# megvii-research/OccDepth

Measured on AMD Instinct MI355X. Metric: frames/sec forward, SemanticKITTI stereo->256x256x32 voxels, higher is better.
Workload: dtype f32 storage and accumulate; matrix arithmetic as 3x bf16 split (hi + mid + lo of both operands, six v_mfma_f32_32x32x16_bf16 per K step; error vs float64 tested within 1.5x of the exact-fp32 kernels', measured 0.8-1.1x) in the head convolutions (K2s3), the small-volume 3x3x3 convolutions and transpo

## Files before the change

include/occdepth_amd.h:

```cpp
#ifndef OCCDEPTH_AMD_H
#define OCCDEPTH_AMD_H

#include <stdint.h>

#ifdef __cplusplus
extern "C" {
#endif

#define OCCD_OK 0
#define OCCD_EINVAL (-1)
#define OCCD_ELAUNCH (-2)
#define OCCD_ENOMEM (-3)

#define OCCD_MAX_VIEWS 4
#define OCCD_MAX_SCALES 4

#define OCCD_ACT_NONE 0
#define OCCD_ACT_RELU 1
#define OCCD_ACT_SIGMOID 2
#define OCCD_ACT_RELU_PRE 3

int occd_abi_version(void);
const char* occd_strerror(int code);

// ... 230 lines not shown
                                    int32_t ths, int32_t act, float slope, int32_t res_first, void* stream);

typedef struct occd_wino_args {
    const float* x;
    const float* upk;
    const float* shift;
    const float* res;
    float* y;
    int32_t batch, cin, cout, H, W;
    int32_t act, res_first, tile_hint;
    float slope;
} occd_wino_args;
int64_t occd_wino_packed_floats(int32_t cout, int32_t cin);
int occd_wino_pack_weights(const float* w, const float* scale, float* upk, int32_t cout, int32_t cin, void* stream);
int occd_wino_conv3x3_fwd(const occd_wino_args* a, void* stream);

int occd_dwconv2d_bwd_data_nchw(const float* gy, const float* w, float* dx, int32_t batch, int32_t C, int32_t H,
                                int32_t W, int32_t k, int32_t stride, int32_t pad_top, int32_t pad_left, int32_t Ho,
                                int32_t Wo, void* stream);
int64_t occd_dwconv2d_bwd_weight_workspace_floats(int32_t batch, int32_t C, int32_t k, int32_t Ho, int32_t Wo);
int occd_dwconv2d_bwd_weight_nchw(const float* x, const float* gy, float* dw, float* workspace, int32_t batch, int32_t C,
                                  int32_t H, int32_t W, int32_t k, int32_t stride, int32_t pad_top, int32_t pad_left,
                                  int32_t Ho, int32_t Wo, void* stream);
int32_t occd_dwconv2d_pool_blocks(int32_t Ho, int32_t Wo);
int occd_dwconv2d_pool_nchw(const float* x, const float* w, const float* scale, const float* shift, float* y,
                            float* pool_part, int32_t batch, int32_t C, int32_t H, int32_t W, int32_t k,
                            int32_t stride, int32_t pad_top, int32_t pad_left, int32_t Ho, int32_t Wo,
                            int32_t act, int64_t x_plane_stride, void* stream);
int occd_plane_reduce(const float* a, const float* b, float* out, int64_t planes, int64_t S, void* stream);
int occd_se_bwd(const float* gg, const float* gate, const float* sums, const float* r, const float* w_reduce,
// ... 249 lines not shown
```

occdepth_amd/csrc/prof.cpp:

```cpp
#include <map>
#include <set>
#include <utility>
#include <mutex>
#include <string>
#include <vector>
#include <cstring>
#include "common.h"

namespace {
struct Rec {
    hipEvent_t e0, e1;
    std::string tag;
    double flops, bytes;
};
std::mutex g_mu;
bool g_on = false;
std::string g_tag;
std::string g_tag_kind;
std::vector<Rec> g_recs;
std::vector<hipEvent_t> g_pool;

hipEvent_t get_event() {
    if (!g_pool.empty()) {
        hipEvent_t e = g_pool.back();
// ... 77 lines not shown
        it->second.ms += ms;
        it->second.flops += r.flops;
        it->second.bytes += r.bytes;
        g_pool.push_back(r.e0);
        g_pool.push_back(r.e1);
    }
    g_recs.clear();
    int n = 0;
    for (auto& kv : agg) {
        if (rows && n < max_rows) rows[n] = kv.second;
        ++n;
    }
    return n;
}

extern "C" int occd_abi_version(void) { return 20; }

extern "C" const char* occd_strerror(int code) {
    switch (code) {
        case OCCD_OK: return "ok";
        case OCCD_EINVAL: return "invalid argument or unsupported geometry";
        case OCCD_ELAUNCH: return "HIP launch/runtime error";
        case OCCD_ENOMEM: return "tile does not fit in LDS";
        default: return "unknown error";
    }
}
```

occdepth_amd/csrc/wino_conv2d.hip:

```cpp
#include <type_traits>
#include "device.h"

namespace {

struct WinoP {
    const float* x;
    const float* upk;
    const float* shift;
    const float* res;
    float* y;
    int B, Cin, Cout, H, W;
    int chunks, nblk, wg_ty, wg_tx, nwg;
    int act, res_first;
    float slope;
};

template <int TWV, int EXP = 0>
__global__ void __launch_bounds__(512, 2) wino3x3_kernel(const WinoP p) {
    constexpr int RW = 32 / TWV;
    constexpr int WGR = 4 * RW;
    constexpr int PR = 2 * WGR + 2;
    constexpr int PC = 2 * TWV + 2;
    constexpr int RS = TWV == 16 ? 48 : 68;
    constexpr int PLANE = PR * RS;
    constexpr int NEL = 8 * PLANE;
    constexpr int NDMA = (NEL + 511) / 512;
    constexpr int PBUF = NDMA * 512;
    constexpr int UBUF = 16 * 256;
    extern __shared__ __attribute__((aligned(16))) float lds[];

// ... 129 lines not shown
            if (EXP != 1 && c + 2 < p.chunks) issue_chunk(c + 2);
            block(pn, (c + 1) & 1, 0, ub, vb, ua, va);
        }
        const int lb = (p.chunks - 1) & 1;
        const float* pl = lds + lb * PBUF + pbase;
        block(pl, lb, 1, ua, va, ub, vb);
        block(pl, lb, 2, ub, vb, ua, va);
        block(pl, lb, 3, ua, va, ub, vb);
        mfma4(ub, vb, 0);
        mfma4(ub, vb, 4);
    };
    if (h0) k_loop(std::integral_constant<int, 0>{});
    else k_loop(std::integral_constant<int, 1>{});
    __syncthreads();

    float* const xchg = lds;
    auto xwrite = [&](auto hc) {
        constexpr int H = decltype(hc)::value;
        constexpr bool h0 = H == 0;
        float* mine = xchg + ((pr * 2 + H) * 64) * 64 + lane;
#pragma unroll
        for (int k = 0; k < 8; ++k)
#pragma unroll
            for (int r8 = 0; r8 < 8; ++r8) mine[(k * 8 + r8) * 64] = h0 ? acc[k][8 + r8] : acc[k][r8];
    };
    if (h0) xwrite(std::integral_constant<int, 0>{});
    else xwrite(std::integral_constant<int, 1>{});
    __syncthreads();
    auto finish = [&](auto hc) {
    constexpr int H = decltype(hc)::value;
    constexpr bool h0 = H == 0;
    const float* theirs = xchg + ((pr * 2 + (1 - H)) * 64) * 64 + lane;

    const int oy0 = 2 * (ty0 + lr), ox = 2 * (tx0 + lc);
    const bool pair = ox + 1 < p.W && (p.W & 1) == 0;
#pragma unroll
    for (int r8 = 0; r8 < 8; ++r8) {
        __builtin_amdgcn_sched_barrier(0);
        const int r = H * 8 + r8;
        const int co = nb * 32 + 8 * (r >> 2) + 4 * kk + (r & 3);
        float m[4][4];
#pragma unroll
        for (int k = 0; k < 8; ++k) {
            const float own = h0 ? acc[k][r8] : acc[k][8 + r8];
            const float oth = theirs[(k * 8 + r8) * 64];
            m[k >> 2][k & 3] = h0 ? own : oth;
            m[2 + (k >> 2)][k & 3] = h0 ? oth : own;
        }
        float s[2][4];
#pragma unroll
        for (int j = 0; j < 4; ++j) {
            s[0][j] = m[0][j] + m[1][j] + m[2][j];
            s[1][j] = m[1][j] - m[2][j] - m[3][j];
        }
        if (co >= p.Cout || ox >= p.W) continue;
        const float sh = p.shift != nullptr ? p.shift[co] : 0.f;
#pragma unroll
        for (int a = 0; a < 2; ++a) {
            const int oy = oy0 + a;
            if (oy >= p.H) continue;
            float y0 = s[a][0] + s[a][1] + s[a][2] + sh;
            float y1 = s[a][1] - s[a][2] - s[a][3] + sh;
            const size_t o = (((size_t)b * p.Cout + co) * p.H + oy) * p.W + ox;
            float r0 = 0.f, r1 = 0.f;
            if (p.res != nullptr) {
                r0 = p.res[o];
                if (ox + 1 < p.W) r1 = p.res[o + 1];
            }
            if (p.res_first) { y0 += r0; y1 += r1; }
            y0 = act2d_exact(y0, p.act, p.slope);
            y1 = act2d_exact(y1, p.act, p.slope);
            if (!p.res_first) { y0 += r0; y1 += r1; }
            if (pair) {
                *(f32x2*)(p.y + o) = f32x2{y0, y1};
            } else {
                p.y[o] = y0;
                if (ox + 1 < p.W) p.y[o + 1] = y1;
            }
        }
    }
    };
    if (h0) finish(std::integral_constant<int, 0>{});
    else finish(std::integral_constant<int, 1>{});
}

__global__ void wino_pack_kernel(const float* __restrict__ w, const float* __restrict__ scale, float* __restrict__ upk,
                                 int cout, int cin, int nblk, long total) {
    const long i = (long)blockIdx.x * blockDim.x + threadIdx.x;
    if (i >= total) return;
    const int j = i & 3, lane = (i >> 2) & 63;
    long t = i >> 8;
    const int blk = t % nblk; t /= nblk;
    const int rec = t & 15;
    const int chunk = (int)(t >> 4);
    const int q = rec >> 2, hh = (rec >> 1) & 1, part = rec & 1;
    const int xi = 8 * hh + 4 * part + j;
    const int co = blk * 32 + (lane & 31), ci = chunk * 8 + (lane >> 5) * 4 + q;
    float out = 0.f;
    if (co < cout && ci < cin) {
        const double G[4][3] = {{1, 0, 0}, {0.5, 0.5, 0.5}, {0.5, -0.5, 0.5}, {0, 0, 1}};
        const float* g = w + ((size_t)co * cin + ci) * 9;
        const int a = xi >> 2, bcol = xi & 3;
        double s = 0.0;
#pragma unroll
        for (int m = 0; m < 3; ++m)
#pragma unroll
            for (int n = 0; n < 3; ++n) s += G[a][m] * (double)g[m * 3 + n] * G[bcol][n];
        if (scale != nullptr) s *= (double)scale[co];
        out = (float)s;
    }
    upk[i] = out;
}

template <int TWV, int EXP = 0>
int launch_wino(const WinoP& p, hipStream_t st) {
    constexpr int RW = 32 / TWV, PR = 2 * 4 * RW + 2, RS = TWV == 16 ? 48 : 68;
    constexpr int PBUF = (8 * PR * RS + 511) / 512 * 512;
    size_t lds = ((size_t)2 * PBUF + 2 * 16 * 256) * sizeof(float);
    const size_t xchg = (size_t)4 * 2 * 64 * 64 * sizeof(float);
    if (lds < xchg) lds = xchg;
    if (occd::ensure_big_lds(reinterpret_cast<const void*>(wino3x3_kernel<TWV, EXP>)) != OCCD_OK) return OCCD_ELAUNCH;
    hipLaunchKernelGGL((wino3x3_kernel<TWV, EXP>), dim3((unsigned)p.nwg), dim3(512), lds, st, p);
    return occd::check_launch();
}

}

extern "C" {

int64_t occd_wino_packed_floats(int32_t cout, int32_t cin) {
    if (cout < 1 || cin < 1) return OCCD_EINVAL;
    return (int64_t)((cin + 7) / 8) * 16 * ((cout + 31) / 32) * 256;
}

int occd_wino_pack_weights(const float* w, const float* scale, float* upk, int32_t cout, int32_t cin, void* stream) {
    if (w == nullptr || upk == nullptr || cout < 1 || cin < 1) return OCCD_EINVAL;
    const long total = occd_wino_packed_floats(cout, cin);
    hipLaunchKernelGGL(wino_pack_kernel, dim3((unsigned)((total + 255) / 256)), dim3(256), 0, (hipStream_t)stream, w,
                       scale, upk, cout, cin, (cout + 31) / 32, total);
    return occd::check_launch();
}

int occd_wino_conv3x3_fwd(const occd_wino_args* a, void* stream) {
    if (a == nullptr || a->x == nullptr || a->upk == nullptr || a->y == nullptr) return OCCD_EINVAL;
    if (a->batch < 1 || a->cin < 1 || a->cout < 1 || a->H < 1 || a->W < 1) return OCCD_EINVAL;
    if (a->act < 0 || a->act > 3) return OCCD_EINVAL;
    if ((double)a->cin * a->H * a->W >= 2147483648.0) return OCCD_EINVAL;
    WinoP p{};
    p.x = a->x; p.upk = a->upk; p.shift = a->shift; p.res = a->res; p.y = a->y;
    p.B = a->batch; p.Cin = a->cin; p.Cout = a->cout; p.H = a->H; p.W = a->W;
    p.chunks = (a->cin + 7) / 8;
    p.nblk = (a->cout + 31) / 32;
    p.act = a->act; p.res_first = a->res_first; p.slope = a->slope;
    const int th = (a->H + 1) / 2, tw = (a->W + 1) / 2;
    const int exp_mode = a->tile_hint / 100;
    const int hint = a->tile_hint % 100;
    int twv = hint == 16 || hint == 32 ? hint : 0;
    if (twv == 0) {
        const long w16 = (long)((tw + 15) / 16) * 16 * ((th + 7) / 8) * 8;
        const long w32 = (long)((tw + 31) / 32) * 32 * ((th + 3) / 4) * 4;
        twv = w32 <= w16 ? 32 : 16;
    }
    const int wgr = twv == 16 ? 8 : 4;
    p.wg_tx = (tw + twv - 1) / twv;
    p.wg_ty = (th + wgr - 1) / wgr;
    const long nwg = (long)p.nblk * p.wg_tx * p.wg_ty * p.B;
    if (nwg > 0x7fffffffL) return OCCD_EINVAL;
    p.nwg = (int)nwg;
    const double tiles = (double)p.B * th * tw;
    occd::ProfScope prof("wino_conv3x3", (hipStream_t)stream, 2.0 * 16 * tiles * p.chunks * 8 * p.nblk * 32,
                         4.0 * p.B * ((double)p.Cin + p.Cout) * p.H * p.W);
#ifdef OCCD_WINO_DEV_VARIANTS
    if (exp_mode == 1) return twv == 16 ? launch_wino<16, 1>(p, (hipStream_t)stream) : launch_wino<32, 1>(p, (hipStream_t)stream);
    if (exp_mode == 2) return twv == 16 ? launch_wino<16, 2>(p, (hipStream_t)stream) : launch_wino<32, 2>(p, (hipStream_t)stream);
#else
    (void)exp_mode;
#endif
    return twv == 16 ? launch_wino<16>(p, (hipStream_t)stream) : launch_wino<32>(p, (hipStream_t)stream);
}

}
```

occdepth_amd/fused.py:

```python
import os

import torch

from . import hip
from .hip import ACT_NONE, ACT_RELU, ACT_RELU_PRE, ACT_SIGMOID, Vox


_warned_eval_with_grad = False


def needs_autograd(module):
    if module.training:
        return True
    if torch.is_grad_enabled():
        global _warned_eval_with_grad
        if not _warned_eval_with_grad:
            _warned_eval_with_grad = True
            import warnings
            warnings.warn("occdepth_amd: eval-mode forward with autograd enabled runs the differentiable ATen path; "
                          "wrap inference in torch.no_grad() to take the HIP eval path", stacklevel=3)
        return True
    return False


# ... 23 lines not shown
    b = bn.bias.float() if bn.bias is not None else torch.zeros_like(inv)
    scale = g * inv
    return scale, b - bn.running_mean.float() * scale


def bn_affine_cached(bn):
    key = _stamp(bn)
    cached = getattr(bn, "_occd_affine", None)
    if cached is None or cached[0] != key:
        scale, shift = _bn_affine(bn, bn.num_features, bn.running_mean.device)
        cached = (key, scale.contiguous(), shift.contiguous())
        bn._occd_affine = cached
    return cached[1], cached[2]


def wino_fused_operands(owner, conv, bn):
    key = _stamp(conv, bn)
    cache = owner.__dict__.setdefault("_fused_cache", {})
    hit = cache.get(id(conv))
    if hit is None or hit[0] != key:
        scale, shift = bn_affine_cached(bn)
        if conv.bias is not None:
            shift = shift + scale * conv.bias.detach().float()
        hit = (key, hip.wino_pack_weights(conv.weight, scale), shift.contiguous())
        cache[id(conv)] = hit
    return hit[1:]


def _pad_bias(bias, cout):
    out = torch.zeros(hip.round_up(cout, 32), device=bias.device, dtype=torch.float32)
    out[:cout] = bias
    return out


def _parse_bf16x3(v):
    v = (v or "0").strip().lower()
    if v in ("0", "", "off", "false"):
        return False
    if v in ("1", "all", "on", "true"):
# ... 336 lines not shown
```

occdepth_amd/hip.py:

```python
import ctypes
import os
from ctypes import POINTER, Structure, c_char, c_char_p, c_double, c_float, c_int32, c_int64, c_uint8, c_void_p

import torch

_HERE = os.path.dirname(os.path.abspath(__file__))
LIB_PATH = os.path.join(_HERE, "libocc_hip.so")

MAX_VIEWS = 4
MAX_SCALES = 4
ACT_NONE, ACT_RELU, ACT_SIGMOID, ACT_RELU_PRE = 0, 1, 2, 3
ABI_VERSION = 20

_c_float_p = POINTER(c_float)


class Conv3dArgs(Structure):
    _fields_ = [
        ("inp", c_void_p), ("wpk", c_void_p), ("bias", c_void_p), ("res1", c_void_p), ("res2", c_void_p),
        ("out", c_void_p),
        ("batch", c_int32),
        ("X", c_int32), ("Y", c_int32), ("Z", c_int32),
        ("cin", c_int32), ("in_cs", c_int32), ("in_coff", c_int32),
        ("cout", c_int32), ("out_cs", c_int32), ("out_coff", c_int32),
        ("res1_cs", c_int32), ("res1_coff", c_int32), ("res2_cs", c_int32), ("res2_coff", c_int32),
        ("kx", c_int32), ("ky", c_int32), ("kz", c_int32),
        ("sx", c_int32), ("sy", c_int32), ("sz", c_int32),
# ... 164 lines not shown
                                        c_int32, c_void_p]),
    "occd_affine_act_nchw": (c_int32, [c_void_p, c_void_p, c_void_p, c_void_p, c_void_p, c_int32, c_int32, c_int64,
                                       c_int32, c_float, c_int32, c_void_p]),
    "occd_dwconv2d_nchw": (c_int32, [c_void_p, c_void_p, c_void_p, c_void_p, c_void_p] + [c_int32] * 11 + [c_void_p]),
    "occd_upsample_bilinear_cat_nchw": (c_int32, [c_void_p, c_void_p, c_void_p] + [c_int32] * 7 + [c_void_p]),
    "occd_swish_bwd": (c_int32, [c_void_p, c_void_p, c_void_p, c_int64, c_void_p]),
    "occd_upconv_gather_skip_nchw": (c_int32, [c_void_p] * 5 + [c_int32] * 7 + [c_int64, c_int64, ctypes.c_float, c_void_p]),
    "occd_upconv_gather_nchw": (c_int32, [c_void_p, c_void_p] + [c_int32] * 6 + [c_int64, c_int64, c_void_p]),
    "occd_wino_input_transform_nchw": (c_int32, [c_void_p, c_void_p, c_int32, c_int32, c_int32, c_int32, c_int32, c_int32,
                                                 c_void_p]),
    "occd_wino_output_transform_nchw": (c_int32, [c_void_p, c_void_p, c_void_p, c_void_p, c_void_p, c_int32, c_int32,
                                                  c_int32, c_int32, c_int32, c_int32, c_int32, c_float, c_int32, c_void_p]),
    "occd_wino_packed_floats": (c_int64, [c_int32, c_int32]),
    "occd_wino_pack_weights": (c_int32, [c_void_p, c_void_p, c_void_p, c_int32, c_int32, c_void_p]),
    "occd_wino_conv3x3_fwd": (c_int32, [POINTER(WinoArgs), c_void_p]),
    "occd_softmax_nchw": (c_int32, [c_void_p, c_void_p, c_int32, c_int32, c_int64, c_void_p]),
    "occd_dwconv2d_bwd_data_nchw": (c_int32, [c_void_p, c_void_p, c_void_p] + [c_int32] * 10 + [c_void_p]),
    "occd_dwconv2d_bwd_weight_workspace_floats": (c_int64, [c_int32] * 5),
    "occd_dwconv2d_bwd_weight_nchw": (c_int32, [c_void_p] * 4 + [c_int32] * 10 + [c_void_p]),
    "occd_dwconv2d_pool_blocks": (c_int32, [c_int32, c_int32]),
    "occd_dwconv2d_pool_nchw": (c_int32, [c_void_p] * 6 + [c_int32] * 11 + [c_int64, c_void_p]),
    "occd_se_gate": (c_int32, [c_void_p] * 7 + [c_int32, c_int32, c_int32, c_int32, c_int64, c_void_p]),
    "occd_pw_packed_floats": (c_int64, [c_int32, c_int32]),
    "occd_pw_pack_weights": (c_int32, [c_void_p, c_void_p, c_void_p, c_int32, c_int32, c_void_p]),
    "occd_pw_conv_fwd": (c_int32, [POINTER(PwArgs), c_void_p]),
    "occd_project_voxels": (c_int32, [c_void_p, c_void_p, c_void_p, c_double] + [c_int32] * 5
                            + [c_void_p, c_void_p, c_void_p, c_void_p]),
    "occd_argmax_channels": (c_int32, [c_void_p, c_int64, c_int32, c_int32, c_int32, c_void_p, c_void_p, c_void_p]),
    "occd_cascade_tail_fwd": (c_int32, [c_void_p, c_void_p, c_void_p] + [c_int32] * 8 + [c_void_p]),
    "occd_conv3d_wgrad_workspace_floats": (c_int64, [POINTER(WgradArgs)]),
# ... 1078 lines not shown
def wino_pack_weights(w, scale=None):
    cout, cin = w.shape[0], w.shape[1]
    if tuple(w.shape[2:]) != (3, 3):
        raise RuntimeError("wino_pack_weights needs a (Cout, Cin, 3, 3) weight")
    n = load().occd_wino_packed_floats(cout, cin)
    if n <= 0:
        raise RuntimeError("occd_wino_packed_floats: bad shape")
    wc = w.detach().float().contiguous()
    upk = torch.empty(n, device=w.device, dtype=torch.float32)
    sc = scale.detach().float().contiguous() if scale is not None else None
    _check(load().occd_wino_pack_weights(_f32(wc, "w"), _f32(sc, "scale") if sc is not None else None,
                                         _f32(upk, "upk"), cout, cin, _stream()), "occd_wino_pack_weights")
    return upk


def conv2d_3x3_fused(x, upk, cout, shift=None, act=None, slope=0.01, res=None, res_first=False, tile_hint=0, out=None):
    if not x.is_contiguous():
        x = x.contiguous()
    B, cin, H, W = x.shape
    y = torch.empty((B, cout, H, W), device=x.device, dtype=torch.float32) if out is None else out
    if res is not None and not res.is_contiguous():
        res = res.contiguous()
    a = WinoArgs()
    a.x, a.upk, a.y = _f32(x, "x"), _f32(upk, "upk"), _f32(y, "y")
    a.shift = _f32(shift, "shift") if shift is not None else None
    a.res = _f32(res, "res") if res is not None else None
    a.batch, a.cin, a.cout, a.H, a.W = B, cin, cout, H, W
    a.act, a.res_first, a.tile_hint, a.slope = ACT2D[act], 1 if res_first else 0, int(tile_hint), float(slope)
    if upk.numel() != load().occd_wino_packed_floats(cout, cin):
        raise RuntimeError("packed Winograd weights do not match (cout, cin)")
    if _PROFILING:
        set_tag("%d>%d @%dx%dx%d" % (cin, cout, B, H, W))
    _check(load().occd_wino_conv3x3_fwd(ctypes.byref(a), _stream()), "occd_wino_conv3x3_fwd")
    return y


def pw_pack_weights(w, scale=None):
    cout, cin = w.shape[0], w.shape[1]
    n = load().occd_pw_packed_floats(cout, cin)
    if n <= 0 or w.numel() != cout * cin:
        raise RuntimeError("pw_pack_weights needs a (Cout, Cin[, 1, 1]) weight")
    wc = w.detach().float().reshape(cout, cin).contiguous()
    wpk = torch.empty(n, device=w.device, dtype=torch.float32)
    sc = scale.detach().float().contiguous() if scale is not None else None
    _check(load().occd_pw_pack_weights(_f32(wc, "w"), _f32(sc, "scale") if sc is not None else None, _f32(wpk, "wpk"),
                                       cout, cin, _stream()), "occd_pw_pack_weights")
    return wpk

# ... 744 lines not shown
```

occdepth_amd/models/unet2d.py:

```python
import os

import torch
import torch.nn as nn
import torch.nn.functional as F

from .. import autograd3d as _ag
from .. import hip
from .. import fused as _fused
from ..fused import _stamp, bn_affine_cached, needs_autograd, wino_fused_operands
from .efficientnet import EfficientNet, pw_operands, pw_wins

MODEL_NAME = "tf_efficientnet_b3_ns"
MODEL_CHANNELS = {
    "tf_efficientnet_b3_ns": [3, 24, 32, 48, 136],
    "tf_efficientnet_b4_ns": [3, 24, 32, 56, 160],
    "tf_efficientnet_b5_ns": [3, 32, 40, 64, 176],
    "tf_efficientnet_b7_ns": [3, 32, 48, 80, 224],
}
NUM_FEATURES = {
    "tf_efficientnet_b3_ns": 1536,
    "tf_efficientnet_b4_ns": 1792,
    "tf_efficientnet_b5_ns": 2048,
    "tf_efficientnet_b7_ns": 2560,
}
# ... 46 lines not shown
            U, scale, shift = self._wino_operands(conv, bn)
            return hip.conv2d_3x3_winograd(f, U, scale, shift, "leaky", act.negative_slope)
        if self.WINOGRAD and C >= self.WINOGRAD_HIRES_MIN_CIN and B * H * W <= self.WINOGRAD_HIRES_PIXELS:
            U, scale, shift = self._wino_operands(conv, bn)
            per_row = 16.0 * B * ((W + 1) // 2) * (C + conv.out_channels) * 4
            rows = max(1, int(self.WINOGRAD_STRIP_MB * 2 ** 20 / per_row))
            return hip.conv2d_3x3_winograd(f, U, scale, shift, "leaky", act.negative_slope, strip_rows=rows)
        return hip.affine_act(conv(f), *bn_affine_cached(bn), "leaky", slope=act.negative_slope)

    UPCONV = os.environ.get("OCCDEPTH_UPCONV", "1") == "1"
    UPCONV_LIB_BELOW = int(os.environ.get("OCCDEPTH_UPCONV_LIB_BELOW", str(1 << 62)))
    UPCONV_FOLD_BELOW = int(os.environ.get("OCCDEPTH_UPCONV_FOLD_BELOW", "0"))
    UPCONV_FUSE_SKIP = os.environ.get("OCCDEPTH_UPCONV_FUSE_SKIP", "1") == "1"

    def _upconv_operands(self, conv, bn, cup):
        key = (_stamp(conv, bn), cup)
        hit = self.__dict__.get("_upconv_cache")
        if hit is None or hit[0] != key:
            scale, shift = bn_affine_cached(bn)
            if conv.bias is not None:
                shift = shift + scale * conv.bias.detach().float()
            w = conv.weight.detach().float()
            cout = w.shape[0]
            w9 = (w[:, :cup] * scale.view(-1, 1, 1, 1)).permute(2, 3, 0, 1).reshape(9 * cout, cup).contiguous()
            wskip = (w[:, cup:] * scale.view(-1, 1, 1, 1)).contiguous()
            hit = (key, hip.pw_pack_weights(w9), hip.matmul_operand(w9, "a"),
                   hip.wino_pack_weights(w[:, cup:].contiguous(), scale), shift.contiguous(), wskip)
            self.__dict__["_upconv_cache"] = hit
        return hit[1:]

    @staticmethod
    def _tap_planes(shape, device):
        return hip.padded_rows(shape, device) if hip.GEMM_X3 else None

    def _first_conv_upconv(self, x, skip, conv, bn, act):
        wpk9, w9, upk_skip, shift, wskip = self._upconv_operands(conv, bn, x.shape[1])
        cout = conv.out_channels
        B, cup, h, w = x.shape
        if B > 1 and B * h * w <= self.UPCONV_FOLD_BELOW:
            z = hip.matmul(w9, x.permute(1, 0, 2, 3).reshape(cup, B * h * w),
                           out=self._tap_planes((9 * cout, B * h * w), x.device)).view(9 * cout, B, h, w)
            batch_inner = True
# ... 210 lines not shown
```

Before: 60.68.

## Add fp16 two-term split Winograd 3x3 conv kernel with per-channel scaling

Adds a Winograd F(2,3) 3x3 convolution kernel that splits the transformed input and weights into fp16 hi/lo pairs. It runs three f16 MFMAs per step instead of the existing fp32-emulating path, with per-output-channel power-of-two scaling to keep the fp16 ranges safe. The old epilogue is factored into a shared exchange/store helper that can apply that scale factor. The fp16 path is on by default through OCCDEPTH_WINO_SPLIT, and a heuristic falls back to the fp32 kernel when the grid is too small to fill the CUs. Packing weights now does a blocking host sync to reject non-finite values, and the fp16 split may lose some accuracy relative to the fp32 path.

```diff
diff --git a/include/occdepth_amd.h b/include/occdepth_amd.h
--- a/include/occdepth_amd.h
+++ b/include/occdepth_amd.h
@@ -268,6 +268,10 @@
 int64_t occd_wino_packed_floats(int32_t cout, int32_t cin);
 int occd_wino_pack_weights(const float* w, const float* scale, float* upk, int32_t cout, int32_t cin, void* stream);
 int occd_wino_conv3x3_fwd(const occd_wino_args* a, void* stream);
+
+int64_t occd_wino_packed_f16x2_bytes(int32_t cout, int32_t cin);
+int occd_wino_pack_weights_f16x2(const float* w, const float* scale, void* upk, int32_t cout, int32_t cin, void* stream);
+int occd_wino_conv3x3_f16x2_fwd(const occd_wino_args* a, void* stream);
 
 int occd_dwconv2d_bwd_data_nchw(const float* gy, const float* w, float* dx, int32_t batch, int32_t C, int32_t H,
                                 int32_t W, int32_t k, int32_t stride, int32_t pad_top, int32_t pad_left, int32_t Ho,
diff --git a/occdepth_amd/csrc/prof.cpp b/occdepth_amd/csrc/prof.cpp
--- a/occdepth_amd/csrc/prof.cpp
+++ b/occdepth_amd/csrc/prof.cpp
@@ -115,7 +115,7 @@
     return n;
 }
 
-extern "C" int occd_abi_version(void) { return 20; }
+extern "C" int occd_abi_version(void) { return 21; }
 
 extern "C" const char* occd_strerror(int code) {
     switch (code) {
diff --git a/occdepth_amd/csrc/wino_conv2d.hip b/occdepth_amd/csrc/wino_conv2d.hip
--- a/occdepth_amd/csrc/wino_conv2d.hip
+++ b/occdepth_amd/csrc/wino_conv2d.hip
@@ -1,4 +1,5 @@
 #include <type_traits>
+#include <vector>
 #include "device.h"
 
 namespace {
@@ -14,6 +15,82 @@
     int act, res_first;
     float slope;
 };
+
+template <int TWV, bool FAC, class P>
+__device__ __forceinline__ void wino_exchange_store(const P& p, const float* fac, f32x16 (&acc)[8], float* xchg, int h, int pr,
+                                                    int lane, int nb, int b, int ty0, int tx0) {
+    constexpr int RW = 32 / TWV;
+    const int li = lane & 31, kk = lane >> 5;
+    const int lr = pr * RW + li / TWV, lc = li % TWV;
+    const bool h0 = h == 0;
+    auto xwrite = [&](auto hc) {
+        constexpr int H = decltype(hc)::value;
+        constexpr bool h0 = H == 0;
+        float* mine = xchg + ((pr * 2 + H) * 64) * 64 + lane;
+#pragma unroll
+        for (int k = 0; k < 8; ++k)
+#pragma unroll
+            for (int r8 = 0; r8 < 8; ++r8) mine[(k * 8 + r8) * 64] = h0 ? acc[k][8 + r8] : acc[k][r8];
+    };
+    if (h0) xwrite(std::integral_constant<int, 0>{});
+    else xwrite(std::integral_constant<int, 1>{});
+    __syncthreads();
+    auto finish = [&](auto hc) {
+    constexpr int H = decltype(hc)::value;
+    constexpr bool h0 = H == 0;
+    const float* theirs = xchg + ((pr * 2 + (1 - H)) * 64) * 64 + lane;
+    const int oy0 = 2 * (ty0 + lr), ox = 2 * (tx0 + lc);
+    const bool pair = ox + 1 < p.W && (p.W & 1) == 0;
+#pragma unroll
+    for (int r8 = 0; r8 < 8; ++r8) {
+        __builtin_amdgcn_sched_barrier(0);
+        const int r = H * 8 + r8;
+        const int co = nb * 32 + 8 * (r >> 2) + 4 * kk + (r & 3);
+        float m[4][4];
+#pragma unroll
+        for (int k = 0; k < 8; ++k) {
+            const float own = h0 ? acc[k][r8] : acc[k][8 + r8];
+            const float oth = theirs[(k * 8 + r8) * 64];
+            m[k >> 2][k & 3] = h0 ? own : oth;
+            m[2 + (k >> 2)][k & 3] = h0 ? oth : own;
+        }
+        float s[2][4];
+#pragma unroll
+        for (int j = 0; j < 4; ++j) {
+            s[0][j] = m[0][j] + m[1][j] + m[2][j];
+            s[1][j] = m[1][j] - m[2][j] - m[3][j];
+        }
+        if (co >= p.Cout || ox >= p.W) continue;
+        const float sh = p.shift != nullptr ? p.shift[co] : 0.f;
+        const float fc = FAC ? fac[co] : 1.f;
+#pragma unroll
+        for (int a = 0; a < 2; ++a) {
+            const int oy = oy0 + a;
+            if (oy >= p.H) continue;
+            float y0 = FAC ? __builtin_fmaf(s[a][0] + s[a][1] + s[a][2], fc, sh) : s[a][0] + s[a][1] + s[a][2] + sh;
+            float y1 = FAC ? __builtin_fmaf(s[a][1] - s[a][2] - s[a][3], fc, sh) : s[a][1] - s[a][2] - s[a][3] + sh;
+            const size_t o = (((size_t)b * p.Cout + co) * p.H + oy) * p.W + ox;
+            float r0 = 0.f, r1 = 0.f;
+            if (p.res != nullptr) {
+                r0 = p.res[o];
+                if (ox + 1 < p.W) r1 = p.res[o + 1];
+            }
+            if (p.res_first) { y0 += r0; y1 += r1; }
+            y0 = act2d_exact(y0, p.act, p.slope);
+            y1 = act2d_exact(y1, p.act, p.slope);
+            if (!p.res_first) { y0 += r0; y1 += r1; }
+            if (pair) {
+                *(f32x2*)(p.y + o) = f32x2{y0, y1};
+            } else {
+                p.y[o] = y0;
+                if (ox + 1 < p.W) p.y[o + 1] = y1;
+            }
+        }
+    }
+    };
+    if (h0) finish(std::integral_constant<int, 0>{});
+    else finish(std::integral_constant<int, 1>{});
+}
 
 template <int TWV, int EXP = 0>
 __global__ void __launch_bounds__(512, 2) wino3x3_kernel(const WinoP p) {
@@ -173,74 +250,7 @@
     else k_loop(std::integral_constant<int, 1>{});
     __syncthreads();
 
-    float* const xchg = lds;
-    auto xwrite = [&](auto hc) {
-        constexpr int H = decltype(hc)::value;
-        constexpr bool h0 = H == 0;
-        float* mine = xchg + ((pr * 2 + H) * 64) * 64 + lane;
-#pragma unroll
-        for (int k = 0; k < 8; ++k)
-#pragma unroll
-            for (int r8 = 0; r8 < 8; ++r8) mine[(k * 8 + r8) * 64] = h0 ? acc[k][8 + r8] : acc[k][r8];
-    };
-    if (h0) xwrite(std::integral_constant<int, 0>{});
-    else xwrite(std::integral_constant<int, 1>{});
-    __syncthreads();
-    auto finish = [&](auto hc) {
-    constexpr int H = decltype(hc)::value;
-    constexpr bool h0 = H == 0;
-    const float* theirs = xchg + ((pr * 2 + (1 - H)) * 64) * 64 + lane;
-
-    const int oy0 = 2 * (ty0 + lr), ox = 2 * (tx0 + lc);
-    const bool pair = ox + 1 < p.W && (p.W & 1) == 0;
-#pragma unroll
-    for (int r8 = 0; r8 < 8; ++r8) {
-        __builtin_amdgcn_sched_barrier(0);
-        const int r = H * 8 + r8;
-        const int co = nb * 32 + 8 * (r >> 2) + 4 * kk + (r & 3);
-        float m[4][4];
-#pragma unroll
-        for (int k = 0; k < 8; ++k) {
-            const float own = h0 ? acc[k][r8] : acc[k][8 + r8];
-            const float oth = theirs[(k * 8 + r8) * 64];
-            m[k >> 2][k & 3] = h0 ? own : oth;
-            m[2 + (k >> 2)][k & 3] = h0 ? oth : own;
-        }
-        float s[2][4];
-#pragma unroll
-        for (int j = 0; j < 4; ++j) {
-            s[0][j] = m[0][j] + m[1][j] + m[2][j];
-            s[1][j] = m[1][j] - m[2][j] - m[3][j];
-        }
-        if (co >= p.Cout || ox >= p.W) continue;
-        const float sh = p.shift != nullptr ? p.shift[co] : 0.f;
-#pragma unroll
-        for (int a = 0; a < 2; ++a) {
-            const int oy = oy0 + a;
-            if (oy >= p.H) continue;
-            float y0 = s[a][0] + s[a][1] + s[a][2] + sh;
-            float y1 = s[a][1] - s[a][2] - s[a][3] + sh;
-            const size_t o = (((size_t)b * p.Cout + co) * p.H + oy) * p.W + ox;
-            float r0 = 0.f, r1 = 0.f;
-            if (p.res != nullptr) {
-                r0 = p.res[o];
-                if (ox + 1 < p.W) r1 = p.res[o + 1];
-            }
-            if (p.res_first) { y0 += r0; y1 += r1; }
-            y0 = act2d_exact(y0, p.act, p.slope);
-            y1 = act2d_exact(y1, p.act, p.slope);
-            if (!p.res_first) { y0 += r0; y1 += r1; }
-            if (pair) {
-                *(f32x2*)(p.y + o) = f32x2{y0, y1};
-            } else {
-                p.y[o] = y0;
-                if (ox + 1 < p.W) p.y[o + 1] = y1;
-            }
-        }
-    }
-    };
-    if (h0) finish(std::integral_constant<int, 0>{});
-    else finish(std::integral_constant<int, 1>{});
+    wino_exchange_store<TWV, false>(p, nullptr, acc, lds, h, pr, lane, nb, b, ty0, tx0);
 }
 
 __global__ void wino_pack_kernel(const float* __restrict__ w, const float* __restrict__ scale, float* __restrict__ upk,
@@ -271,6 +281,241 @@
     upk[i] = out;
 }
 
+constexpr int kWinoStageExp = 1;
+typedef _Float16 f16x2 __attribute__((ext_vector_type(2)));
+
+struct WinoHP {
+    const float* x;
+    const uint16_t* upk;
+    const float* fac;
+    const float* shift;
+    const float* res;
+    float* y;
+    int B, Cin, Cout, H, W;
+    int chunks, nblk, wg_ty, wg_tx, nwg;
+    int act, res_first;
+    float slope;
+};
+
+__device__ __forceinline__ void split2_f16x2(float a, float b, uint32_t& hi, uint32_t& lo) {
+    asm("" : "+v"(a));
+    asm("" : "+v"(b));
+    const f16x2 h = __builtin_convertvector((f32x2){a, b}, f16x2);
+    float r0 = __builtin_fmaf((float)h[0], -2048.f, a * 2048.f);
+    float r1 = __builtin_fmaf((float)h[1], -2048.f, b * 2048.f);
+    asm("" : "+v"(r0));
+    asm("" : "+v"(r1));
+    hi = __builtin_bit_cast(uint32_t, h);
+    lo = __builtin_bit_cast(uint32_t, __builtin_convertvector((f32x2){r0, r1}, f16x2));
+}
+
+template <int TWV>
+__global__ void __launch_bounds__(512, 2) wino3x3_f16x2_kernel(const WinoHP p) {
+    constexpr int RW = 32 / TWV;
+    constexpr int WGR = 4 * RW;
+    constexpr int PR = 2 * WGR + 2;
+    constexpr int PC = 2 * TWV + 2;
+    constexpr int RS = TWV == 16 ? 48 : 68;
+    constexpr int PLANE = PR * RS;
+    constexpr int NEL = 8 * PLANE;
+    constexpr int NDMA = (NEL + 511) / 512;
+    constexpr int PBUF = NDMA * 512;
+    constexpr int UOFF = 4 * PBUF;
+    extern __shared__ __attribute__((aligned(16))) float lds[];
+
+    const int tid = threadIdx.x;
+    const int lane = tid & 63;
+    const int wave = __builtin_amdgcn_readfirstlane(tid >> 6);
+    const int pr = wave & 3, h = wave >> 2;
+    const int li = lane & 31, kk = lane >> 5;
+
+    const uint32_t bid = xcd_remap(blockIdx.x, p.nwg);
+    const int nb = bid % p.nblk;
+    uint32_t t = bid / p.nblk;
+    const int bx = t % p.wg_tx;
+    t /= p.wg_tx;
+    const int by = t % p.wg_ty;
+    const int b = t / p.wg_ty;
+    const int ty0 = by * WGR, tx0 = bx * TWV;
+    const int gy0 = 2 * ty0 - 1, gx0 = 2 * tx0 - 1;
+
+    const size_t plane_hw = (size_t)p.H * p.W;
+    uint32_t voff[NDMA];
+#pragma unroll
+    for (int i = 0; i < NDMA; ++i) {
+        const int e = (wave * NDMA + i) * 64 + lane;
+        const int cin = e / PLANE, rem = e - cin * PLANE;
+        const int row = rem / RS, col = rem - row * RS;
+        const int gy = gy0 + row, gx = gx0 + col;
+        const bool ok = e < NEL && col < PC && (unsigned)gy < (unsigned)p.H && (unsigned)gx < (unsigned)p.W;
+        voff[i] = ok ? (uint32_t)((cin * plane_hw + (size_t)gy * p.W + gx) * 4) : 0xFFFFFFF0u;
+    }
+    const float* const xb = p.x + (size_t)b * p.Cin * plane_hw;
+    const uint16_t* const ubase = p.upk + (size_t)nb * 512 + lane * 8;
+    const size_t u_rec = (size_t)p.nblk * 512;
+
+    auto issue_patch = [&](int c) {
+#pragma unroll
+        for (int s = 0; s < 2; ++s) {
+            const int ch0 = c * 16 + s * 8, left = p.Cin - ch0;
+            const auto rsrc = __builtin_amdgcn_make_buffer_rsrc((void*)(xb + (size_t)(left > 0 ? ch0 : 0) * plane_hw), 0,
+                                                                left > 0 ? (uint32_t)((size_t)left * plane_hw * 4) : 0u, 0x00020000);
+            float* pdst = lds + ((c & 1) * 2 + s) * PBUF + wave * NDMA * 64;
+#pragma unroll
+            for (int i = 0; i < NDMA; ++i)
+                __builtin_amdgcn_raw_ptr_buffer_load_lds(rsrc, pdst + i * 64, 4, voff[i], 0, 0, 0);
+        }
+    };
+    auto issue_u = [&](int c) {
+        float* udst = lds + UOFF + wave * 4 * 256;
+        const uint16_t* usrc = ubase + ((size_t)c * 32 + wave * 4) * u_rec;
+#pragma unroll
+        for (int j = 0; j < 4; ++j) __builtin_amdgcn_global_load_lds(usrc + (size_t)j * u_rec, udst + j * 256, 16, 0, 0);
+    };
+
+    const int lr = pr * RW + li / TWV, lc = li % TWV;
+    const int pbase = kk * PBUF + (2 * lr + h) * RS + 2 * lc;
+
+    asm volatile("" ::"a"(0.f));
+    f32x16 acc[8];
+#pragma unroll
+    for (int k = 0; k < 8; ++k)
+#pragma unroll
+        for (int r = 0; r < 16; ++r) acc[k][r] = 0.f;
+
+    static_assert(kWinoStageExp == 1, "the transform below stages 2 V");
+    auto row_v = [&](auto hc, auto ic, const float* pl, uint32_t (&vh)[4][4], uint32_t (&vl)[4][4]) {
+        constexpr int H = decltype(hc)::value, I = decltype(ic)::value;
+        constexpr int RA = H == 0 ? I : 1 - I, RB = H == 1 && I == 0 ? 0 : 2;
+        constexpr bool ADD = H == 0 && I == 1;
+#pragma unroll
+        for (int m = 0; m < 4; ++m) {
+            float v[2][4];
+#pragma unroll
+            for (int e = 0; e < 2; ++e) {
+                const float* pq = pl + (2 * m + e) * PLANE;
+                const f32x2 a0 = *(const f32x2*)(pq + RA * RS), a1 = *(const f32x2*)(pq + RA * RS + 2);
+                const f32x2 b0 = *(const f32x2*)(pq + RB * RS), b1 = *(const f32x2*)(pq + RB * RS + 2);
+                float ra[4] = {a0.x, a0.y, a1.x, a1.y};
+#pragma unroll
+                for (int j = 0; j < 4; ++j) asm("" : "+v"(ra[j]));
+                const float t0 = ADD ? ra[0] + b0.x : ra[0] - b0.x, t1 = ADD ? ra[1] + b0.y : ra[1] - b0.y;
+                const float t2 = ADD ? ra[2] + b1.x : ra[2] - b1.x, t3 = ADD ? ra[3] + b1.y : ra[3] - b1.y;
+                const float u1 = 2.f * t1, u2 = 2.f * t2;
+                v[e][0] = __builtin_fmaf(2.f, t0, -u2);
+                v[e][1] = u1 + u2;
+                v[e][2] = u2 - u1;
+                v[e][3] = __builtin_fmaf(-2.f, t3, u1);
+            }
+#pragma unroll
+            for (int j = 0; j < 4; ++j) split2_f16x2(v[0][j], v[1][j], vh[j][m], vl[j][m]);
+        }
+    };
+    const u32x4* const ul = (const u32x4*)(lds + UOFF) + (h * 16 * 64 + lane);
+    auto row_m = [&](auto ic, const uint32_t (&vh)[4][4], const uint32_t (&vl)[4][4]) {
+        constexpr int I = decltype(ic)::value;
+#pragma unroll
+        for (int j = 0; j < 4; j += 2) {
+            f16x8 uh[2], ulo[2], us[2], bh[2], bl[2];
+#pragma unroll
+            for (int e = 0; e < 2; ++e) {
+                uh[e] = __builtin_bit_cast(f16x8, ul[(2 * (4 * I + j + e)) * 64]);
+                ulo[e] = __builtin_bit_cast(f16x8, ul[(2 * (4 * I + j + e) + 1) * 64]);
+                us[e] = uh[e] * (_Float16)(1.f / 2048.f);
+                bh[e] = __builtin_bit_cast(f16x8, (u32x4){vh[j + e][0], vh[j + e][1], vh[j + e][2], vh[j + e][3]});
+                bl[e] = __builtin_bit_cast(f16x8, (u32x4){vl[j + e][0], vl[j + e][1], vl[j + e][2], vl[j + e][3]});
+            }
+#pragma unroll
+            for (int e = 0; e < 2; ++e)
+                acc[4 * I + j + e] = __builtin_amdgcn_mfma_f32_32x32x16_f16(ulo[e], bh[e], acc[4 * I + j + e], 0, 0, 0);
+#pragma unroll
+            for (int e = 0; e < 2; ++e)
+                acc[4 * I + j + e] = __builtin_amdgcn_mfma_f32_32x32x16_f16(us[e], bl[e], acc[4 * I + j + e], 0, 0, 0);
+#pragma unroll
+            for (int e = 0; e < 2; ++e)
+                acc[4 * I + j + e] = __builtin_amdgcn_mfma_f32_32x32x16_f16(uh[e], bh[e], acc[4 * I + j + e], 0, 0, 0);
+        }
+    };
+    using I0 = std::integral_constant<int, 0>;
+    using I1 = std::integral_constant<int, 1>;
+
+    const bool h0 = h == 0;
+    issue_patch(0);
+    __syncthreads();
+    for (int c = 0; c < p.chunks; ++c) {
+        issue_u(c);
+        if (c + 1 < p.chunks) issue_patch(c + 1);
+        const float* pl = lds + (c & 1) * 2 * PBUF + pbase;
+        uint32_t ah[4][4], al[4][4], bh[4][4], bl[4][4];
+        if (h0) row_v(I0{}, I0{}, pl, ah, al);
+        else row_v(I1{}, I0{}, pl, ah, al);
+        __syncthreads();
+        row_m(I0{}, ah, al);
+        if (h0) row_v(I0{}, I1{}, pl, bh, bl);
+        else row_v(I1{}, I1{}, pl, bh, bl);
+        row_m(I1{}, bh, bl);
+        __syncthreads();
+    }
+
+    int tid_e = threadIdx.x;
+    asm volatile("" : "+v"(tid_e));
+    wino_exchange_store<TWV, true>(p, p.fac, acc, lds, h, pr, tid_e & 63, nb, b, ty0, tx0);
+}
+
+__device__ __forceinline__ double wino_u_f64(const float* g, int xi) {
+    const double G[4][3] = {{1, 0, 0}, {0.5, 0.5, 0.5}, {0.5, -0.5, 0.5}, {0, 0, 1}};
+    const int a = xi >> 2, bcol = xi & 3;
+    double s = 0.0;
+#pragma unroll
+    for (int m = 0; m < 3; ++m)
+#pragma unroll
+        for (int n = 0; n < 3; ++n) s += G[a][m] * (double)g[m * 3 + n] * G[bcol][n];
+    return s;
+}
+
+__global__ void wino_f16x2_scale_kernel(const float* __restrict__ w, const float* __restrict__ scale, float* __restrict__ fac,
+                                        int cout, int cin, int nblk) {
+    const int co = blockIdx.x * blockDim.x + threadIdx.x;
+    if (co >= nblk * 32) return;
+    double m = 0.0;
+    bool bad = false;
+    if (co < cout) {
+        const double sc = scale != nullptr ? (double)scale[co] : 1.0;
+        for (int ci = 0; ci < cin; ++ci)
+            for (int xi = 0; xi < 16; ++xi) {
+                const double v = fabs(wino_u_f64(w + ((size_t)co * cin + ci) * 9, xi) * sc);
+                if (!(v <= 3.0e38)) bad = true;
+                m = fmax(m, v);
+            }
+    }
+    int e = 0;
+    const bool ok = m > 0.0 && !bad;
+    if (ok) frexp(m, &e);
+    const int k = ok ? min(max(14 - e, -100), 100) : 0;
+    fac[co] = bad ? __builtin_nanf("") : ldexpf(1.f, -(k + kWinoStageExp));
+}
+
+__global__ void wino_pack_f16x2_kernel(const float* __restrict__ w, const float* __restrict__ scale,
+                                       const float* __restrict__ fac, uint16_t* __restrict__ upk, int cout, int cin, int nblk,
+                                       long total) {
+    const long i = (long)blockIdx.x * blockDim.x + threadIdx.x;
+    if (i >= total) return;
+    const int j = i & 7, lane = (i >> 3) & 63;
+    long t = i >> 9;
+    const int blk = t % nblk; t /= nblk;
+    const int img = t & 1, xi = (t >> 1) & 15;
+    const int chunk = (int)(t >> 5);
+    const int co = blk * 32 + (lane & 31), ci = chunk * 16 + (lane >> 5) * 8 + j;
+    float v = 0.f;
+    if (co < cout && ci < cin) {
+        double s = wino_u_f64(w + ((size_t)co * cin + ci) * 9, xi);
+        if (scale != nullptr) s *= (double)scale[co];
+        v = (float)(s * (double)(ldexpf(1.f, -kWinoStageExp) / fac[co]));
+    }
+    const _Float16 hi = (_Float16)v;
+    upk[i] = __builtin_bit_cast(uint16_t, img == 0 ? hi : (_Float16)(v - (float)hi));
+}
+
 template <int TWV, int EXP = 0>
 int launch_wino(const WinoP& p, hipStream_t st) {
     constexpr int RW = 32 / TWV, PR = 2 * 4 * RW + 2, RS = TWV == 16 ? 48 : 68;
@@ -283,6 +528,46 @@
     return occd::check_launch();
 }
 
+template <int TWV>
+int launch_wino_f16x2(const WinoHP& p, hipStream_t st) {
+    constexpr int RW = 32 / TWV, PR = 2 * 4 * RW + 2, RS = TWV == 16 ? 48 : 68;
+    constexpr int PBUF = (8 * PR * RS + 511) / 512 * 512;
+    size_t lds = ((size_t)4 * PBUF + 32 * 256) * sizeof(float);
+    const size_t xchg = (size_t)4 * 2 * 64 * 64 * sizeof(float);
+    if (lds < xchg) lds = xchg;
+    if (occd::ensure_big_lds(reinterpret_cast<const void*>(wino3x3_f16x2_kernel<TWV>)) != OCCD_OK) return OCCD_ELAUNCH;
+    hipLaunchKernelGGL((wino3x3_f16x2_kernel<TWV>), dim3((unsigned)p.nwg), dim3(512), lds, st, p);
+    return occd::check_launch();
+}
+
+template <class P>
+int wino_geometry(const occd_wino_args* a, int cin_step, P& p) {
+    if (a == nullptr || a->x == nullptr || a->upk == nullptr || a->y == nullptr) return OCCD_EINVAL;
+    if (a->batch < 1 || a->cin < 1 || a->cout < 1 || a->H < 1 || a->W < 1) return OCCD_EINVAL;
+    if (a->act < 0 || a->act > 3) return OCCD_EINVAL;
+    if ((double)a->cin * a->H * a->W >= 2147483648.0) return OCCD_EINVAL;
+    p.x = a->x; p.shift = a->shift; p.res = a->res; p.y = a->y;
+    p.B = a->batch; p.Cin = a->cin; p.Cout = a->cout; p.H = a->H; p.W = a->W;
+    p.chunks = (a->cin + cin_step - 1) / cin_step;
+    p.nblk = (a->cout + 31) / 32;
+    p.act = a->act; p.res_first = a->res_first; p.slope = a->slope;
+    const int th = (a->H + 1) / 2, tw = (a->W + 1) / 2;
+    const int hint = a->tile_hint % 100;
+    int twv = hint == 16 || hint == 32 ? hint : 0;
+    if (twv == 0) {
+        const long w16 = (long)((tw + 15) / 16) * 16 * ((th + 7) / 8) * 8;
+        const long w32 = (long)((tw + 31) / 32) * 32 * ((th + 3) / 4) * 4;
+        twv = w32 <= w16 ? 32 : 16;
+    }
+    const int wgr = twv == 16 ? 8 : 4;
+    p.wg_tx = (tw + twv - 1) / twv;
+    p.wg_ty = (th + wgr - 1) / wgr;
+    const long nwg = (long)p.nblk * p.wg_tx * p.wg_ty * p.B;
+    if (nwg > 0x7fffffffL) return OCCD_EINVAL;
+    p.nwg = (int)nwg;
+    return twv;
+}
+
 }
 
 extern "C" {
@@ -301,31 +586,12 @@
 }
 
 int occd_wino_conv3x3_fwd(const occd_wino_args* a, void* stream) {
-    if (a == nullptr || a->x == nullptr || a->upk == nullptr || a->y == nullptr) return OCCD_EINVAL;
-    if (a->batch < 1 || a->cin < 1 || a->cout < 1 || a->H < 1 || a->W < 1) return OCCD_EINVAL;
-    if (a->act < 0 || a->act > 3) return OCCD_EINVAL;
-    if ((double)a->cin * a->H * a->W >= 2147483648.0) return OCCD_EINVAL;
     WinoP p{};
-    p.x = a->x; p.upk = a->upk; p.shift = a->shift; p.res = a->res; p.y = a->y;
-    p.B = a->batch; p.Cin = a->cin; p.Cout = a->cout; p.H = a->H; p.W = a->W;
-    p.chunks = (a->cin + 7) / 8;
-    p.nblk = (a->cout + 31) / 32;
-    p.act = a->act; p.res_first = a->res_first; p.slope = a->slope;
+    const int twv = wino_geometry(a, 8, p);
+    if (twv < 0) return twv;
+    p.upk = a->upk;
     const int th = (a->H + 1) / 2, tw = (a->W + 1) / 2;
     const int exp_mode = a->tile_hint / 100;
-    const int hint = a->tile_hint % 100;
-    int twv = hint == 16 || hint == 32 ? hint : 0;
-    if (twv == 0) {
-        const long w16 = (long)((tw + 15) / 16) * 16 * ((th + 7) / 8) * 8;
-        const long w32 = (long)((tw + 31) / 32) * 32 * ((th + 3) / 4) * 4;
-        twv = w32 <= w16 ? 32 : 16;
-    }
-    const int wgr = twv == 16 ? 8 : 4;
-    p.wg_tx = (tw + twv - 1) / twv;
-    p.wg_ty = (th + wgr - 1) / wgr;
-    const long nwg = (long)p.nblk * p.wg_tx * p.wg_ty * p.B;
-    if (nwg > 0x7fffffffL) return OCCD_EINVAL;
-    p.nwg = (int)nwg;
     const double tiles = (double)p.B * th * tw;
     occd::ProfScope prof("wino_conv3x3", (hipStream_t)stream, 2.0 * 16 * tiles * p.chunks * 8 * p.nblk * 32,
                          4.0 * p.B * ((double)p.Cin + p.Cout) * p.H * p.W);
@@ -338,4 +604,42 @@
     return twv == 16 ? launch_wino<16>(p, (hipStream_t)stream) : launch_wino<32>(p, (hipStream_t)stream);
 }
 
-}
+int64_t occd_wino_packed_f16x2_bytes(int32_t cout, int32_t cin) {
+    if (cout < 1 || cin < 1) return OCCD_EINVAL;
+    const int64_t nblk = (cout + 31) / 32;
+    return (int64_t)((cin + 15) / 16) * 32 * nblk * 512 * 2 + nblk * 32 * 4;
+}
+
+int occd_wino_pack_weights_f16x2(const float* w, const float* scale, void* upk, int32_t cout, int32_t cin, void* stream) {
+    if (w == nullptr || upk == nullptr || cout < 1 || cin < 1) return OCCD_EINVAL;
+    const int nblk = (cout + 31) / 32;
+    const long total = (long)((cin + 15) / 16) * 32 * nblk * 512;
+    float* fac = reinterpret_cast<float*>(static_cast<uint16_t*>(upk) + total);
+    hipLaunchKernelGGL(wino_f16x2_scale_kernel, dim3((unsigned)nblk), dim3(32), 0, (hipStream_t)stream, w, scale, fac, cout,
+                       cin, nblk);
+    hipLaunchKernelGGL(wino_pack_f16x2_kernel, dim3((unsigned)((total + 255) / 256)), dim3(256), 0, (hipStream_t)stream, w,
+                       scale, fac, static_cast<uint16_t*>(upk), cout, cin, nblk, total);
+    const int rc = occd::check_launch();
+    if (rc != OCCD_OK) return rc;
+    std::vector<float> host((size_t)nblk * 32);
+    if (hipMemcpyAsync(host.data(), fac, host.size() * sizeof(float), hipMemcpyDeviceToHost, (hipStream_t)stream) != hipSuccess ||
+        hipStreamSynchronize((hipStream_t)stream) != hipSuccess)
+        return OCCD_ELAUNCH;
+    for (float f : host)
+        if (f != f) return OCCD_EINVAL;
+    return OCCD_OK;
+}
+
+int occd_wino_conv3x3_f16x2_fwd(const occd_wino_args* a, void* stream) {
+    WinoHP p{};
+    const int twv = wino_geometry(a, 16, p);
+    if (twv < 0) return twv;
+    p.upk = reinterpret_cast<const uint16_t*>(a->upk);
+    p.fac = reinterpret_cast<const float*>(p.upk + (size_t)p.chunks * 32 * p.nblk * 512);
+    const double tiles = (double)p.B * ((a->H + 1) / 2) * ((a->W + 1) / 2);
+    occd::ProfScope prof("wino_conv3x3_f16x2", (hipStream_t)stream, 2.0 * 16 * tiles * ((a->cin + 7) / 8) * 8 * p.nblk * 32,
+                         4.0 * p.B * ((double)p.Cin + p.Cout) * p.H * p.W);
+    return twv == 16 ? launch_wino_f16x2<16>(p, (hipStream_t)stream) : launch_wino_f16x2<32>(p, (hipStream_t)stream);
+}
+
+}
diff --git a/occdepth_amd/fused.py b/occdepth_amd/fused.py
--- a/occdepth_amd/fused.py
+++ b/occdepth_amd/fused.py
@@ -61,15 +61,42 @@
     return cached[1], cached[2]
 
 
+def _parse_wino_split(v):
+    v = (v or "f16x2").strip().lower()
+    if v not in ("f16x2", "fp32"):
+        raise ValueError(f"OCCDEPTH_WINO_SPLIT={v!r}: expected f16x2 or fp32")
+    return v
+
+
+WINO_SPLIT = _parse_wino_split(os.environ.get("OCCDEPTH_WINO_SPLIT", "f16x2"))
+
+
+def set_wino_split(v):
+    global WINO_SPLIT
+    WINO_SPLIT = _parse_wino_split(v)
+
+
+def wino_pack(w, scale=None):
+    f32 = hip.wino_pack_weights(w, scale)
+    if WINO_SPLIT != "f16x2" or not w.is_cuda:
+        return f32
+    try:
+        upk = hip.wino_pack_weights_f16x2(w, scale)
+    except ValueError:
+        return f32
+    upk.f32 = f32
+    return upk
+
+
 def wino_fused_operands(owner, conv, bn):
-    key = _stamp(conv, bn)
+    key = (_stamp(conv, bn), WINO_SPLIT)
     cache = owner.__dict__.setdefault("_fused_cache", {})
     hit = cache.get(id(conv))
     if hit is None or hit[0] != key:
         scale, shift = bn_affine_cached(bn)
         if conv.bias is not None:
             shift = shift + scale * conv.bias.detach().float()
-        hit = (key, hip.wino_pack_weights(conv.weight, scale), shift.contiguous())
+        hit = (key, wino_pack(conv.weight, scale), shift.contiguous())
         cache[id(conv)] = hit
     return hit[1:]
 
diff --git a/occdepth_amd/hip.py b/occdepth_amd/hip.py
--- a/occdepth_amd/hip.py
+++ b/occdepth_amd/hip.py
@@ -10,7 +10,7 @@
 MAX_VIEWS = 4
 MAX_SCALES = 4
 ACT_NONE, ACT_RELU, ACT_SIGMOID, ACT_RELU_PRE = 0, 1, 2, 3
-ABI_VERSION = 20
+ABI_VERSION = 21
 
 _c_float_p = POINTER(c_float)
 
@@ -205,6 +205,9 @@
     "occd_wino_packed_floats": (c_int64, [c_int32, c_int32]),
     "occd_wino_pack_weights": (c_int32, [c_void_p, c_void_p, c_void_p, c_int32, c_int32, c_void_p]),
     "occd_wino_conv3x3_fwd": (c_int32, [POINTER(WinoArgs), c_void_p]),
+    "occd_wino_packed_f16x2_bytes": (c_int64, [c_int32, c_int32]),
+    "occd_wino_pack_weights_f16x2": (c_int32, [c_void_p, c_void_p, c_void_p, c_int32, c_int32, c_void_p]),
+    "occd_wino_conv3x3_f16x2_fwd": (c_int32, [POINTER(WinoArgs), c_void_p]),
     "occd_softmax_nchw": (c_int32, [c_void_p, c_void_p, c_int32, c_int32, c_int64, c_void_p]),
     "occd_dwconv2d_bwd_data_nchw": (c_int32, [c_void_p, c_void_p, c_void_p] + [c_int32] * 10 + [c_void_p]),
     "occd_dwconv2d_bwd_weight_workspace_floats": (c_int64, [c_int32] * 5),
@@ -1313,6 +1316,47 @@
     return upk
 
 
+class WinoF16x2:
+
+    __slots__ = ("image", "cout", "cin", "f32")
+
+    def __init__(self, image, cout, cin, f32=None):
+        self.image, self.cout, self.cin, self.f32 = image, cout, cin, f32
+
+
+_CU_COUNT = {}
+
+
+def _cu_count(device):
+    n = _CU_COUNT.get(device)
+    if n is None:
+        n = _CU_COUNT[device] = torch.cuda.get_device_properties(device).multi_processor_count
+    return n
+
+
+def wino_f16x2_wins(B, cin, cout, H, W, device=None):
+    tiles = B * ((H + 1) // 2) * ((W + 1) // 2)
+    return ((cout + 31) // 32) * ((tiles + 127) // 128) >= _cu_count(torch.cuda.current_device() if device is None else device)
+
+
+def wino_pack_weights_f16x2(w, scale=None):
+    cout, cin = w.shape[0], w.shape[1]
+    if tuple(w.shape[2:]) != (3, 3):
+        raise RuntimeError("wino_pack_weights_f16x2 needs a (Cout, Cin, 3, 3) weight")
+    n = load().occd_wino_packed_f16x2_bytes(cout, cin)
+    if n <= 0:
+        raise RuntimeError("occd_wino_packed_f16x2_bytes: bad shape")
+    wc = w.detach().float().contiguous()
+    sc = scale.detach().float().contiguous() if scale is not None else None
+    image = torch.empty(n, device=w.device, dtype=torch.uint8)
+    rc = load().occd_wino_pack_weights_f16x2(_f32(wc, "w"), _f32(sc, "scale") if sc is not None else None,
+                                             _ptr(image, "upk"), cout, cin, _stream())
+    if rc == -1:
+        raise ValueError("wino_pack_weights_f16x2: non-finite weights (keep the float32 image of wino_pack_weights)")
+    _check(rc, "occd_wino_pack_weights_f16x2")
+    return WinoF16x2(image, cout, cin)
+
+
 def conv2d_3x3_fused(x, upk, cout, shift=None, act=None, slope=0.01, res=None, res_first=False, tile_hint=0, out=None):
     if not x.is_contiguous():
         x = x.contiguous()
@@ -1320,17 +1364,24 @@
     y = torch.empty((B, cout, H, W), device=x.device, dtype=torch.float32) if out is None else out
     if res is not None and not res.is_contiguous():
         res = res.contiguous()
+    if isinstance(upk, WinoF16x2) and upk.f32 is not None and not wino_f16x2_wins(B, cin, cout, H, W, x.device):
+        upk = upk.f32
+    split = isinstance(upk, WinoF16x2)
     a = WinoArgs()
-    a.x, a.upk, a.y = _f32(x, "x"), _f32(upk, "upk"), _f32(y, "y")
+    a.x, a.y = _f32(x, "x"), _f32(y, "y")
+    a.upk = _ptr(upk.image, "upk") if split else _f32(upk, "upk")
     a.shift = _f32(shift, "shift") if shift is not None else None
     a.res = _f32(res, "res") if res is not None else None
     a.batch, a.cin, a.cout, a.H, a.W = B, cin, cout, H, W
     a.act, a.res_first, a.tile_hint, a.slope = ACT2D[act], 1 if res_first else 0, int(tile_hint), float(slope)
-    if upk.numel() != load().occd_wino_packed_floats(cout, cin):
+    if (upk.cout, upk.cin) != (cout, cin) if split else upk.numel() != load().occd_wino_packed_floats(cout, cin):
         raise RuntimeError("packed Winograd weights do not match (cout, cin)")
     if _PROFILING:
         set_tag("%d>%d @%dx%dx%d" % (cin, cout, B, H, W))
-    _check(load().occd_wino_conv3x3_fwd(ctypes.byref(a), _stream()), "occd_wino_conv3x3_fwd")
+    if split:
+        _check(load().occd_wino_conv3x3_f16x2_fwd(ctypes.byref(a), _stream()), "occd_wino_conv3x3_f16x2_fwd")
+    else:
+        _check(load().occd_wino_conv3x3_fwd(ctypes.byref(a), _stream()), "occd_wino_conv3x3_fwd")
     return y
 
 
diff --git a/occdepth_amd/models/unet2d.py b/occdepth_amd/models/unet2d.py
--- a/occdepth_amd/models/unet2d.py
+++ b/occdepth_amd/models/unet2d.py
@@ -84,7 +84,7 @@
     UPCONV_FUSE_SKIP = os.environ.get("OCCDEPTH_UPCONV_FUSE_SKIP", "1") == "1"
 
     def _upconv_operands(self, conv, bn, cup):
-        key = (_stamp(conv, bn), cup)
+        key = (_stamp(conv, bn), cup, _fused.WINO_SPLIT)
         hit = self.__dict__.get("_upconv_cache")
         if hit is None or hit[0] != key:
             scale, shift = bn_affine_cached(bn)
@@ -95,7 +95,7 @@
             w9 = (w[:, :cup] * scale.view(-1, 1, 1, 1)).permute(2, 3, 0, 1).reshape(9 * cout, cup).contiguous()
             wskip = (w[:, cup:] * scale.view(-1, 1, 1, 1)).contiguous()
             hit = (key, hip.pw_pack_weights(w9), hip.matmul_operand(w9, "a"),
-                   hip.wino_pack_weights(w[:, cup:].contiguous(), scale), shift.contiguous(), wskip)
+                   _fused.wino_pack(w[:, cup:].contiguous(), scale), shift.contiguous(), wskip)
             self.__dict__["_upconv_cache"] = hit
         return hit[1:]
 
```

Result: faster. 62.79, median of 6 (+3.5%).
